# malcolmgreaves/deequ

Hardware: AMD Instinct MI355X
Metric: rows/sec (whole node) for fused 16-col profile scan; % of HBM peak BW (higher is better)
Workload: dtype f64+int64+utf8; 1 GPU; C5 fused 16-col profile scan (8 f64 + 4 i64 + 4 utf8, 10% nulls) + state merge + incremental StateLoader append; rows_per_gpu=1000000000, chunk_rows=125000000, analyzers=93, parallelism=row-shard x1

## Files before the change

### deequ_amd/csrc/dq_kernels.hip

```cpp
#include <hip/hip_runtime.h>

#include <cstdint>
#include <type_traits>

#include "dq_device.h"
#include "dq_hash.h"
#include "dq_decimal.h"
#include "dq_lane.h"
#include "dq_shift.h"

namespace dq {

#define DQ_DEC_TABLE static __constant__ const
#include "dq_dec_tables.inc"
#undef DQ_DEC_TABLE
__device__ __forceinline__ DecTab dec_dev_tab() { return DecTab{kDecP10Lo, kDecP10Hi, kDecRcpHi, kDecRcpLo}; }

typedef uint32_t u32x4 __attribute__((ext_vector_type(4)));

__device__ __forceinline__ uint32_t ld32(const uint8_t* base, int64_t a) {
  return *reinterpret_cast<const uint32_t*>(base + a);
}
__device__ __forceinline__ uint32_t read4(const uint8_t* base, int64_t pos) {
  int64_t a = pos & ~int64_t(3);
// ... 60 lines not shown

__device__ __forceinline__ void hll_update_if(int32_t* regs, uint64_t x, bool b) {
  atomicMax(&regs[(uint32_t)(x >> 55)], b ? hll_q_exact(x) : -1);
}

__device__ __forceinline__ int32_t ffbh_raw(uint32_t x) {
  int32_t r;
  asm("v_ffbh_u32 %0, %1" : "=v"(r) : "v"(x));
  return r;
}

struct HllKey {
  uint32_t addr;
  int32_t q;
};
__device__ __forceinline__ HllKey hll_key_from_fmix(uint64_t b) {
  const uint32_t bl = (uint32_t)b, bh = (uint32_t)(b >> 32);
  const uint32_t hi = __umulhi(bl, (uint32_t)XP3) + bl * (uint32_t)(XP3 >> 32) + bh * (uint32_t)XP3;
  return {(hi >> 21) & 0x7FCu, ffbh_raw(hi << 9)};
}
__device__ __forceinline__ HllKey hll_key_long(uint64_t v) { return hll_key_from_fmix(xxh64_long_head(v)); }
__device__ __forceinline__ HllKey hll_key_int(uint32_t v) { return hll_key_from_fmix(xxh64_int_head(v)); }


struct ColStats {
  double n, mean, m2, sum;
  int64_t isum, count, nan_count;
  double fmin, fmax;
  int64_t pinf, ninf;
  int64_t isum_hi;
};

__device__ __forceinline__ void stats_init(ColStats& s) {
  s.n = 0.0; s.mean = 0.0; s.m2 = 0.0; s.sum = 0.0;
// ... 170 lines not shown
    asm volatile(
        "s_and_saveexec_b64 %[save], %[ma]\n\t"
        "v_add_f64 %[d], %[x], -%[sh]\n\t"
        "v_add_f64 %[sd], %[sd], %[d]\n\t"
        "v_fma_f64 %[sdd], %[d], %[d], %[sdd]\n\t"
        "s_and_b64 exec, %[save], %[mb]\n\t"
        "v_min_f64 %[lo], %[lo], %[x]\n\t"
        "v_max_f64 %[hi], %[hi], %[x]\n\t"
        "s_mov_b64 exec, %[save]"
        : [sd] "+v"(a.sd), [sdd] "+v"(a.sdd), [lo] "+v"(lo), [hi] "+v"(hi), [d] "=&v"(d), [save] "=&s"(save)
        : [x] "v"(x), [sh] "s"(shift), [ma] "s"(ma), [mb] "s"(mb)
        : "scc");
  }
}

template <int KIND, bool STATS, bool HLL>
__device__ __forceinline__ void numeric_block(const double (&x)[8], const uint64_t (&bits)[8], const uint64_t (&m)[8],
                                              double shift, ColStats& s, LaneMoments& a, int32_t* regs, int32_t& qmin) {
#pragma unroll
  for (int j = 0; j < 8; ++j) {
    if (STATS) masked_moments<!ck_float(KIND), false>(a, s.fmin, s.fmax, x[j], bits[j], shift, m[j], m[j]);
    if (HLL) {
      const HllKey key = ck_bytes(KIND) <= 4 ? hll_key_int((uint32_t)bits[j]) : hll_key_long(bits[j]);
      qmin = min(qmin, key.q);
      if (lane_bit(m[j])) atomicMax(reinterpret_cast<int32_t*>(reinterpret_cast<char*>(regs) + key.addr), key.q);
    }
  }
  if (HLL) {
    if (__builtin_amdgcn_ballot_w64(qmin < 0) != 0) {
#pragma unroll 1
      for (int j = 0; j < 8; ++j) {
        if (lane_bit(m[j])) hll_update(regs, ck_bytes(KIND) <= 4 ? xxh64_int((uint32_t)bits[j]) : xxh64_long(bits[j]));
      }
      qmin = 0;
    }
  }
}

template <int KIND, bool STATS, bool HLL>
__device__ __forceinline__ void float_block_checked(__amdgpu_buffer_rsrc_t vr, const uint32_t* validity,
                                                    const uint32_t* mask, int64_t base, int32_t rem, int32_t vo,
                                                    double shift, ColStats& s, LaneMoments& a, int32_t* regs,
                                                    int64_t& cnt_w, int64_t& nan_v, int64_t& pinf_v, int64_t& ninf_v) {
  constexpr bool kF32 = KIND == CK_F32;
// ... 36 lines not shown
        else hll_update(regs, kF32 ? xxh64_int((uint32_t)b) : xxh64_long(b));
      }
    }
  }
}

template <int K> struct KindT { using T = double; };
template <> struct KindT<CK_I64> { using T = int64_t; };
template <> struct KindT<CK_I32> { using T = int32_t; };
template <> struct KindT<CK_F32> { using T = float; };
template <> struct KindT<CK_I16> { using T = int16_t; };
template <> struct KindT<CK_I8> { using T = int8_t; };

template <int KIND, bool STATS, bool HLL>
__device__ void numeric_range(const void* values, const uint32_t* validity, const uint32_t* mask,
                              int64_t row0, int64_t row1, ColStats& s, int32_t* regs) {
  using T = typename KindT<KIND>::T;
  constexpr bool kLazy = ck_float(KIND) && STATS;
  const int lane = threadIdx.x & 63;
  const int wave = __builtin_amdgcn_readfirstlane(threadIdx.x >> 6);
  const T* v = reinterpret_cast<const T*>(values);
  const __amdgpu_buffer_rsrc_t vr = __builtin_amdgcn_make_buffer_rsrc(
      const_cast<T*>(v + row0), (short)0, (int)((row1 - row0) * (int64_t)sizeof(T)), 0x00020000);
  int64_t nan_v = 0, pinf_v = 0, ninf_v = 0;
  int64_t cnt_w = 0;
  LaneMoments a{0.0, 0.0, 0};
  const double shift =
      STATS ? range_shift(validity, mask, row0, row1, lane, [=](int64_t r) { return range_value<KIND>(vr, r - row0); }) : 0.0;
  int32_t qmin = 0;
  const int32_t nr = (int32_t)(row1 - row0);
  for (int32_t rb = 0; rb < nr; rb += kRowsPerIter) {
    const int64_t base = row0 + rb + wave * 512;
    const int32_t rem = nr - rb - wave * 512;
    const bool full = rb + kRowsPerIter <= nr;
    uint64_t bits[8], m[8];
    double x[8];
    const int32_t vo = (rb + wave * 512 + lane) * (int32_t)sizeof(T);
#pragma unroll
    for (int j = 0; j < 8; ++j) {
      if constexpr (sizeof(T) == 8) {
        const auto w2 = __builtin_amdgcn_raw_buffer_load_b64(vr, vo + j * 512, 0, 2 );
        bits[j] = ((uint64_t)w2[1] << 32) | w2[0];
        if (KIND == CK_F64) x[j] = __builtin_bit_cast(double, bits[j]);
        else x[j] = __builtin_fma((double)(int32_t)w2[1], 4294967296.0, (double)w2[0]);
      } else if constexpr (KIND == CK_F32) {
        const uint32_t w = __builtin_amdgcn_raw_buffer_load_b32(vr, vo + j * 256, 0, 2 );
        bits[j] = w;
        x[j] = (double)__builtin_bit_cast(float, w);
      } else {
        int32_t w;
        if constexpr (sizeof(T) == 4) w = (int32_t)__builtin_amdgcn_raw_buffer_load_b32(vr, vo + j * 256, 0, 2 );
        else if constexpr (sizeof(T) == 2) w = (int16_t)__builtin_amdgcn_raw_buffer_load_b16(vr, vo + j * 128, 0, 2 );
        else w = (int8_t)__builtin_amdgcn_raw_buffer_load_b8(vr, vo + j * 64, 0, 2 );
        bits[j] = (uint64_t)(int64_t)w;
        x[j] = (double)w;
      }
    }
    block_masks(validity, mask, base, rem, full, m);
    uint64_t nf_any = 0;
    if constexpr (ck_float(KIND) && !kLazy) {
#pragma unroll
      for (int j = 0; j < 8; ++j) nf_any |= __builtin_amdgcn_ballot_w64(!__builtin_isfinite(x[j])) & m[j];
    }
    if (ck_float(KIND) && !kLazy && nf_any != 0) {
      float_block_checked<KIND, STATS, HLL>(vr, validity, mask, base, rem, vo, shift, s, a, regs, cnt_w, nan_v, pinf_v,
                                            ninf_v);
    } else {
#pragma unroll
      for (int j = 0; j < 8; ++j) cnt_w += __builtin_popcountll(m[j]);
      numeric_block<KIND, STATS, HLL>(x, bits, m, shift, s, a, regs, qmin);
    }
  }
  if constexpr (kLazy) {
    __shared__ int32_t redo;
    if (threadIdx.x == 0) redo = 0;
    __syncthreads();
    const bool bad = !__builtin_isfinite(a.sd) || !__builtin_isfinite(a.sdd);
    if (__builtin_amdgcn_ballot_w64(bad) != 0 && lane == 0) redo = 1;
    __syncthreads();
    if (redo) {
      if (HLL) {
        for (int i = threadIdx.x; i < 512; i += kBlock) regs[i] = -1;
      }
      stats_init(s);
      a = LaneMoments{0.0, 0.0, 0};
      cnt_w = 0;
      __syncthreads();
// ... 599 lines not shown
    c += __popc(bits);
  }
  s.count += c;
}

template <int KIND, bool STATS, bool HLL>
__device__ void run_numeric(const ColTask& t, const ScanCols& cols, const ScanBitmaps& bm, int64_t row0, int64_t row1,
                            ColStats& s, int32_t* regs) {
  const uint32_t* mask = t.where >= 0 ? reinterpret_cast<const uint32_t*>(bm.where_bits[t.where]) : nullptr;
  numeric_range<KIND, STATS, HLL>(cols.values[t.col], cols.validity[t.col], mask, row0, row1, s, regs);
}

template <int V, bool LONG>
__device__ __forceinline__ void run_variant(const ColTask& t, const ScanCols& cols, const uint32_t* mask, int64_t row0,
                                            int64_t row1, int64_t n_rows, ColStats& s, int32_t* regs,
                                            const uint64_t* p5, uint32_t* dq, uint32_t* rare, uint32_t* cls) {
  const void* v = cols.values[t.col];
  const uint32_t* val = cols.validity[t.col];
  if constexpr (V == CV_VALIDITY) validity_range(val, mask, row0, row1, s);
  else if constexpr (V == CV_F64_S) numeric_range<CK_F64, true, false>(v, val, mask, row0, row1, s, regs);
  else if constexpr (V == CV_F64_SH) numeric_range<CK_F64, true, true>(v, val, mask, row0, row1, s, regs);
  else if constexpr (V == CV_F64_H) numeric_range<CK_F64, false, true>(v, val, mask, row0, row1, s, regs);
  else if constexpr (V == CV_I64_S) numeric_range<CK_I64, true, false>(v, val, mask, row0, row1, s, regs);
  else if constexpr (V == CV_I64_SH) numeric_range<CK_I64, true, true>(v, val, mask, row0, row1, s, regs);
  else if constexpr (V == CV_I64_H) numeric_range<CK_I64, false, true>(v, val, mask, row0, row1, s, regs);
  else if constexpr (V == CV_I32_S) numeric_range<CK_I32, true, false>(v, val, mask, row0, row1, s, regs);
  else if constexpr (V == CV_I32_SH) numeric_range<CK_I32, true, true>(v, val, mask, row0, row1, s, regs);
  else if constexpr (V == CV_I32_H) numeric_range<CK_I32, false, true>(v, val, mask, row0, row1, s, regs);
  else if constexpr (V == CV_F32_S) numeric_range<CK_F32, true, false>(v, val, mask, row0, row1, s, regs);
  else if constexpr (V == CV_F32_SH) numeric_range<CK_F32, true, true>(v, val, mask, row0, row1, s, regs);
  else if constexpr (V == CV_F32_H) numeric_range<CK_F32, false, true>(v, val, mask, row0, row1, s, regs);
  else if constexpr (V == CV_I16_S) numeric_range<CK_I16, true, false>(v, val, mask, row0, row1, s, regs);
  else if constexpr (V == CV_I16_SH) numeric_range<CK_I16, true, true>(v, val, mask, row0, row1, s, regs);
  else if constexpr (V == CV_I16_H) numeric_range<CK_I16, false, true>(v, val, mask, row0, row1, s, regs);
  else if constexpr (V == CV_I8_S) numeric_range<CK_I8, true, false>(v, val, mask, row0, row1, s, regs);
  else if constexpr (V == CV_I8_SH) numeric_range<CK_I8, true, true>(v, val, mask, row0, row1, s, regs);
  else if constexpr (V == CV_I8_H) numeric_range<CK_I8, false, true>(v, val, mask, row0, row1, s, regs);
  else if constexpr (V == CV_F64_D) float_dtype_range(reinterpret_cast<const double*>(v), val, mask, row0, row1, s);
  else if constexpr (V == CV_F32_D) float_dtype_range(reinterpret_cast<const float*>(v), val, mask, row0, row1, s);
  else if constexpr (V == CV_BOOL) bool_range(reinterpret_cast<const uint32_t*>(v), val, mask, row0, row1, s, regs);
  else if constexpr (V == CV_D128_S) decimal_range<true, false, false>(v, val, mask, row0, row1, s, regs, t.arg);
  else if constexpr (V == CV_D128_SH) decimal_range<true, true, false>(v, val, mask, row0, row1, s, regs, t.arg);
  else if constexpr (V == CV_D128_H) decimal_range<false, true, false>(v, val, mask, row0, row1, s, regs, t.arg);
  else if constexpr (V == CV_D128_D) decimal_range<false, false, true>(v, val, mask, row0, row1, s, regs, t.arg);
  else if constexpr (V == CV_UTF8_H || V == CV_UTF8_D || V == CV_UTF8_HD)
    utf8_range<int32_t, V != CV_UTF8_D, V != CV_UTF8_H, LONG>(
        reinterpret_cast<const uint8_t*>(v), reinterpret_cast<const int32_t*>(cols.offsets[t.col]), val, mask, row0,
        row1, n_rows, s, regs, p5, dq, rare, cls);
  else
    utf8_range<int64_t, V != CV_LUTF8_D, V != CV_LUTF8_H, LONG>(
        reinterpret_cast<const uint8_t*>(v), reinterpret_cast<const int64_t*>(cols.offsets[t.col]), val, mask, row0,
        row1, n_rows, s, regs, p5, dq, rare, cls);
// ... 5 lines not shown
#ifndef DQ_NUM_WAVES
#define DQ_NUM_WAVES 6
#endif
template <int V, bool LONG>
constexpr int kMinWaves = V == CV_UTF8_H && !LONG && DQ_STR_CLS ? 5
                          : V == CV_UTF8_H && DQ_STR_WAVES > 0 ? DQ_STR_WAVES
                          : (V == CV_F64_SH || V == CV_I64_SH) && DQ_NUM_WAVES > 0 ? DQ_NUM_WAVES
                          : V == CV_LUTF8_H && LONG ? 5
                                                    : 1;

template <int V, bool LONG = false>
__global__ __launch_bounds__(kBlock) __attribute__((amdgpu_waves_per_eu(kMinWaves<V, LONG>))) void dq_column_scan(const ColTask* __restrict__ tasks, int32_t ntasks,
                                                         int32_t part_base, ScanCols cols, ScanBitmaps bm,
                                                         int64_t n_rows, int64_t rows_per_range,
                                                         ColPartial* __restrict__ partials,
                                                         uint32_t* __restrict__ hll_acc) {
  constexpr bool kHll = !(V == CV_VALIDITY || V == CV_F64_S || V == CV_I64_S || V == CV_I32_S || V == CV_F64_D ||
                         V == CV_UTF8_D || V == CV_LUTF8_D || V == CV_F32_S || V == CV_I16_S || V == CV_I8_S ||
                         V == CV_F32_D || V == CV_BOOL || V == CV_D128_S || V == CV_D128_D);
  constexpr bool kBool = V == CV_BOOL;
  constexpr bool kStr = V == CV_UTF8_H || V == CV_LUTF8_H || V == CV_UTF8_HD || V == CV_LUTF8_HD;
  __shared__ int32_t regs[kHll ? 512 : 2];
  __shared__ uint64_t p5[kStr ? 256 : 1];
  constexpr uint32_t kDCap = DQ_STR_CLS && (V == CV_UTF8_H || V == CV_LUTF8_H) && !LONG ? kDefCapCls : kDefCap;
  __shared__ uint32_t dfq[kStr ? kWaves * kDefFields * kDCap : 1];
  __shared__ uint32_t rare[kStr ? kWaves : 1];
  constexpr bool kCls = DQ_STR_CLS && (V == CV_UTF8_H || V == CV_LUTF8_H) && !LONG;
  __shared__ __attribute__((aligned(16))) uint32_t clsbuf[kCls ? kWaves * kClsWords : 4];
  __shared__ ColStats red[kWaves];
  const int32_t ti = blockIdx.x % ntasks;
  const int32_t range = blockIdx.x / ntasks;
// ... 6 lines not shown
    __syncthreads();
  }
  if constexpr (kHll) {
    for (int i = threadIdx.x; i < 512; i += kBlock) regs[i] = -1;
    if constexpr (kStr) {
      p5[threadIdx.x] = (uint64_t)threadIdx.x * XP5;
      if (threadIdx.x < kWaves) rare[threadIdx.x] = 0;
    }
    __syncthreads();
  }
  ColStats s;
  stats_init(s);
  const uint32_t* mask = t.where >= 0 ? reinterpret_cast<const uint32_t*>(bm.where_bits[t.where]) : nullptr;
  const int32_t wv = kStr ? __builtin_amdgcn_readfirstlane(threadIdx.x >> 6) : 0;
  run_variant<V, LONG>(t, cols, mask, row0, row1, n_rows, s, regs, p5, dfq + wv * kDefFields * kDCap, rare + wv,
                       clsbuf + (kCls ? wv * kClsWords : 0));
  block_reduce_store(s, partials + (size_t)(part_base + ti) * kMaxWG + range, red);
  if constexpr (kStr) {
    if (threadIdx.x == 0 && bm.rare_rows) {
      uint32_t r = 0;
      for (int w = 0; w < kWaves; ++w) r += rare[w];
      if (r) atomicAdd(reinterpret_cast<unsigned long long*>(bm.rare_rows + part_base + ti), (unsigned long long)r);
    }
  }
  if constexpr (kBool) {
    if (threadIdx.x == 0 && t.hll_slot >= 0) {
      uint32_t* dst = hll_acc + ((size_t)t.hll_slot * kHllCopies + (blockIdx.x % kHllCopies)) * 512;
      for (int b = 0; b < 2; ++b) {
        if (!regs[b]) continue;
        const uint64_t x = xxh64_int(b == 0 ? 1u : 0u);
        atomicMax(dst + (uint32_t)(x >> 55), (uint32_t)(hll_q_exact(x) + 1));
// ... 505 lines not shown
        pred_logic_op(ow, S, sp, lane);
      }
    }
    pred_block_out(S, s_ctr, n_counters, s_bmroot, n_bitmaps, bm, wr, inr, n_rows, lane);
  }
  pred_counters_out(pred_lds, wave_words, prog, acc);
}

__global__ __launch_bounds__(kBlock) void dq_finalize(int32_t ncol, int32_t nranges_col,
                                                      const ColPartial* __restrict__ col_part,
                                                      ColPartial* __restrict__ col_acc, int32_t npair, int32_t nranges_pair,
                                                      const CorrPartial* __restrict__ pair_part,
                                                      CorrPartial* __restrict__ pair_acc, int32_t has_pred,
                                                      int32_t nranges_pred, const PredPartial* __restrict__ pred_part,
                                                      PredPartial* __restrict__ pred_acc, FinRanges fr,
                                                      int64_t* __restrict__ rare_dev, int64_t* rare_host) {
  __shared__ ColStats cs[kBlock];
  __shared__ CorrStats ps[kBlock];
  const int b = blockIdx.x, tid = threadIdx.x;
  if (b < ncol) {
    int32_t nr = nranges_col;
    for (int i = 0; i < fr.n; ++i)
      if (b >= fr.first[i] && b < fr.end[i]) nr = fr.nr[i];
    ColStats s;
    stats_init(s);
    for (int r = tid; r < nr; r += kBlock) stats_merge(s, stats_load(col_part + (size_t)b * kMaxWG + r));
    cs[tid] = s;
    __syncthreads();
    for (int stride = kBlock / 2; stride >= 1; stride >>= 1) {
      if (tid < stride) { ColStats a = cs[tid]; stats_merge(a, cs[tid + stride]); cs[tid] = a; }
      __syncthreads();
// ... 15 lines not shown
      CorrStats o = {q.n, q.xa, q.ya, q.ck, q.xm, q.ym};
      corr_merge(s, o);
    }
    ps[tid] = s;
    __syncthreads();
    for (int stride = kBlock / 2; stride >= 1; stride >>= 1) {
      if (tid < stride) { CorrStats a = ps[tid]; corr_merge(a, ps[tid + stride]); ps[tid] = a; }
      __syncthreads();
    }
    if (tid == 0) {
      CorrPartial& q = pair_acc[p];
      CorrStats acc = {q.n, q.xa, q.ya, q.ck, q.xm, q.ym};
      corr_merge(acc, ps[0]);
      q.n = acc.n; q.xa = acc.xa; q.ya = acc.ya; q.ck = acc.ck; q.xm = acc.xm; q.ym = acc.ym;
    }
  } else if (has_pred) {
    static_assert(kBlock % kMaxCounters == 0, "counter layout");
    constexpr int G = kBlock / kMaxCounters;
    __shared__ int64_t st[G][kMaxCounters], sn[G][kMaxCounters];
    const int c = tid % kMaxCounters, g = tid / kMaxCounters;
    int64_t t = 0, nn = 0;
    for (int r = g; r < nranges_pred; r += G) { t += pred_part[r].t[c]; nn += pred_part[r].nn[c]; }
    st[g][c] = t;
    sn[g][c] = nn;
    __syncthreads();
    if (tid < kMaxCounters) {
      int64_t a = pred_acc->t[tid], b = pred_acc->nn[tid];
      for (int k = 0; k < G; ++k) { a += st[k][tid]; b += sn[k][tid]; }
      pred_acc->t[tid] = a;
      pred_acc->nn[tid] = b;
// ... 18 lines not shown
hipError_t launch_pred_scan(const PredProgram* prog, const ScanCols& cols, const ScanBitmaps& bm, int64_t n_rows,
                            int64_t rows_per_range, int32_t nranges, PredPartial* acc, int32_t lds_bytes, hipStream_t st,
                            bool has_regex) {
  if (has_regex)
    hipLaunchKernelGGL(dq_pred_scan<true>, dim3(nranges), dim3(kBlock), (size_t)lds_bytes, st, prog, cols, bm, n_rows,
                       rows_per_range, acc);
  else
    hipLaunchKernelGGL(dq_pred_scan<false>, dim3(nranges), dim3(kBlock), (size_t)lds_bytes, st, prog, cols, bm, n_rows,
                       rows_per_range, acc);
  return hipGetLastError();
}

template <int V>
static void launch_v(const ColTask* tasks, int32_t ntasks, int32_t part_base, const ScanCols& cols,
                     const ScanBitmaps& bm, int64_t n_rows, int64_t rows_per_range, int32_t nranges,
                     ColPartial* partials, uint32_t* hll_acc, bool long_str, hipStream_t st) {
  constexpr bool kStrHll = V == CV_UTF8_H || V == CV_LUTF8_H || V == CV_UTF8_HD || V == CV_LUTF8_HD;
  if constexpr (kStrHll) {
    if (long_str) {
      hipLaunchKernelGGL((dq_column_scan<V, true>), dim3((uint32_t)ntasks * (uint32_t)nranges), dim3(kBlock), 0, st,
                         tasks, ntasks, part_base, cols, bm, n_rows, rows_per_range, partials, hll_acc);
      return;
    }
  }
  hipLaunchKernelGGL(dq_column_scan<V>, dim3((uint32_t)ntasks * (uint32_t)nranges), dim3(kBlock), 0, st, tasks, ntasks,
                     part_base, cols, bm, n_rows, rows_per_range, partials, hll_acc);
}

hipError_t launch_column_scan(int32_t variant, const ColTask* tasks, int32_t ntasks, int32_t part_base,
                              const ScanCols& cols, const ScanBitmaps& bm, int64_t n_rows, int64_t rows_per_range,
                              int32_t nranges, ColPartial* partials, uint32_t* hll_acc, bool long_str, hipStream_t st) {
#define DQ_V(V)                                                                                            \
  case V:                                                                                                  \
    launch_v<V>(tasks, ntasks, part_base, cols, bm, n_rows, rows_per_range, nranges, partials, hll_acc, long_str, \
                st);                                                                                       \
    break;
  switch (variant) {
    DQ_V(CV_VALIDITY) DQ_V(CV_F64_S) DQ_V(CV_F64_SH) DQ_V(CV_F64_H) DQ_V(CV_I64_S) DQ_V(CV_I64_SH) DQ_V(CV_I64_H)
    DQ_V(CV_I32_S) DQ_V(CV_I32_SH) DQ_V(CV_I32_H) DQ_V(CV_UTF8_H) DQ_V(CV_LUTF8_H)
    DQ_V(CV_UTF8_D) DQ_V(CV_UTF8_HD) DQ_V(CV_LUTF8_D) DQ_V(CV_LUTF8_HD) DQ_V(CV_F64_D)
    DQ_V(CV_F32_S) DQ_V(CV_F32_SH) DQ_V(CV_F32_H) DQ_V(CV_I16_S) DQ_V(CV_I16_SH) DQ_V(CV_I16_H)
    DQ_V(CV_I8_S) DQ_V(CV_I8_SH) DQ_V(CV_I8_H) DQ_V(CV_F32_D) DQ_V(CV_BOOL)
    DQ_V(CV_D128_S) DQ_V(CV_D128_SH) DQ_V(CV_D128_H) DQ_V(CV_D128_D)
    default: return hipErrorInvalidValue;
  }
#undef DQ_V
  return hipGetLastError();
}


hipError_t launch_finalize(int32_t ncol, int32_t nranges_col, const ColPartial* col_part, ColPartial* col_acc,
                           int32_t npair, int32_t nranges_pair, const CorrPartial* pair_part, CorrPartial* pair_acc,
                           int32_t has_pred, int32_t nranges_pred, const PredPartial* pred_part, PredPartial* pred_acc,
                           const FinRanges& fr, int64_t* rare_dev, int64_t* rare_host, hipStream_t st) {
  const uint32_t nb = (uint32_t)(ncol + npair + (has_pred ? 1 : 0));
  if (nb == 0) return hipSuccess;
  hipLaunchKernelGGL(dq_finalize, dim3(nb), dim3(kBlock), 0, st, ncol, nranges_col, col_part, col_acc, npair,
                     nranges_pair, pair_part, pair_acc, has_pred, nranges_pred, pred_part, pred_acc, fr, rare_dev,
                     rare_host);
  return hipGetLastError();
}

hipError_t launch_init_acc(ColPartial* col_acc, int32_t ncol, CorrPartial* pair_acc, int32_t npair, int64_t* rare_dev,
                           hipStream_t st) {
  const int n = ncol > npair ? ncol : npair;
  if (n == 0) return hipSuccess;
  hipLaunchKernelGGL(dq_init_acc, dim3((n + 255) / 256), dim3(256), 0, st, col_acc, ncol, pair_acc, npair, rare_dev);
  return hipGetLastError();
}

}
```

### deequ_amd/csrc/dq_plan.cpp

```cpp
#include <hip/hip_runtime.h>

#include <algorithm>
#include <chrono>
#include <cmath>
#include <cstdarg>
#include <cstdio>
#include <cstdlib>
#include <cstring>
#include <functional>
#include <iterator>
#include <limits>
#include <map>
#include <memory>
#include <string>
#include <tuple>
#include <vector>

#include "dq_device.h"
#include "dq_internal.h"
#include "dq_pred_jit.h"

#ifndef DQ_MIN_RANGE_ROWS
#define DQ_MIN_RANGE_ROWS 16384
#endif
// ... 6 lines not shown
#ifndef DQ_PAIR_ONE_ROUND
#define DQ_PAIR_ONE_ROUND 1
#endif
#ifndef DQ_PRED_WGS
#define DQ_PRED_WGS 2048
#endif
#include "dq_regex.h"

namespace dq {

hipError_t launch_pred_scan(const PredProgram* prog, const ScanCols& cols, const ScanBitmaps& bm, int64_t n_rows,
                            int64_t rows_per_range, int32_t nranges, PredPartial* acc, int32_t lds_bytes, hipStream_t st,
                            bool has_regex);
hipError_t launch_column_scan(int32_t variant, const ColTask* tasks, int32_t ntasks, int32_t part_base,
                              const ScanCols& cols, const ScanBitmaps& bm, int64_t n_rows, int64_t rows_per_range,
                              int32_t nranges, ColPartial* partials, uint32_t* hll_acc, bool long_str, hipStream_t st);
hipError_t launch_pair_scan(const PairWG* wgs, int32_t nwg, const ScanCols& cols, const ScanBitmaps& bm,
                            const uint32_t* ones, int64_t n_rows, int64_t rows_per_range, int32_t nranges,
                            CorrPartial* pair_part, ColPartial* col_part, int32_t* redo, bool all_f64, bool ring,
                            bool minmax, hipStream_t st);
hipError_t pair_scan_residency(bool all_f64, bool ring, bool minmax, int32_t* per_cu);
hipError_t launch_finalize(int32_t ncol, int32_t nranges_col, const ColPartial* col_part, ColPartial* col_acc,
                           int32_t npair, int32_t nranges_pair, const CorrPartial* pair_part, CorrPartial* pair_acc,
                           int32_t has_pred, int32_t nranges_pred, const PredPartial* pred_part, PredPartial* pred_acc, const FinRanges& fr, int64_t* rare_dev, int64_t* rare_host,
                           hipStream_t st);
hipError_t launch_init_acc(ColPartial* col_acc, int32_t ncol, CorrPartial* pair_acc, int32_t npair, int64_t* rare_dev,
                           hipStream_t st);

static thread_local char g_err[1024] = "";
static thread_local bool g_capacity = false;

dq_status set_error(dq_status code, const char* fmt, ...) {
  va_list ap;
  va_start(ap, fmt);
  std::vsnprintf(g_err, sizeof(g_err), fmt, ap);
  va_end(ap);
  return code;
}

static dq_status cap_error(const char* fmt, ...) {
// ... 546 lines not shown
  int32_t* d_pair_redo = nullptr;
  char* h_stage = nullptr;
  int64_t* d_rare_dev = nullptr;
  int64_t* h_rare = nullptr;
  int64_t* d_rare = nullptr;
  std::vector<uint8_t> str_long;
  int32_t str_path = 0;
  int64_t prev_rows = 0;
  size_t h_stage_bytes = 0;
  PredProgram* d_prog = nullptr;
  ColPartial* d_col_part = nullptr;
  CorrPartial* d_pair_part = nullptr;
  PredPartial* d_pred_part = nullptr;
  ColPartial* d_col_acc = nullptr;
  uint32_t* d_hll_acc = nullptr;
  CorrPartial* d_pair_acc = nullptr;
  PredPartial* d_pred_acc = nullptr;
  uint64_t* d_where_bits[kMaxWhere] = {nullptr};
  int64_t where_cap_words = 0;
  uint32_t* d_ones = nullptr;
  int64_t ones_cap_words = 0;

  int64_t total_rows = 0;
  int64_t next_chunk = 0;

  bool timing = false;
  std::vector<hipEvent_t> ev_pool;
  struct Pending { int kernel; hipEvent_t a, b; };
  std::vector<Pending> pending;
  static constexpr int kTimers = 16 + kNumVariants;
// ... 40 lines not shown
  HIP_TRY(fn());
  if (p->timing) {
    HIP_TRY(hipEventRecord(b, st));
    p->pending.push_back({kernel, a, b});
  }
  return DQ_OK;
}

static dq_status free_plan_mem(dq_plan* p) {
  for (auto& q : p->pending) { p->ev_pool.push_back(q.a); p->ev_pool.push_back(q.b); }
  p->pending.clear();
  for (hipEvent_t e : p->ev_pool) (void)hipEventDestroy(e);
  p->ev_pool.clear();
  void* ptrs[] = {p->d_col_tasks, p->d_pair_tasks, p->d_pair_wgs, p->d_prog, p->d_col_part, p->d_pair_part,
                  p->d_pred_part, p->d_col_acc, p->d_hll_acc, p->d_pair_acc, p->d_pred_acc, p->d_regex, p->d_pair_redo,
                  p->d_rare_dev};
  for (void* q : ptrs)
    if (q) (void)hipFree(q);
  for (int i = 0; i < kMaxWhere; ++i)
    if (p->d_where_bits[i]) (void)hipFree(p->d_where_bits[i]);
  if (p->d_ones) (void)hipFree(p->d_ones);
  if (p->h_rare) (void)hipHostFree(p->h_rare);
  p->h_rare = p->d_rare = nullptr;
  if (p->h_stage) (void)hipHostFree(p->h_stage);
  p->h_stage = nullptr;
  p->h_stage_bytes = 0;
  return DQ_OK;
}

static dq_status reset_acc(dq_plan* p) {
  HIP_TRY(launch_init_acc(p->d_col_acc, (int32_t)p->col_tasks.size(), p->d_pair_acc, (int32_t)p->pair_tasks.size(),
                          p->d_rare_dev, p->stream));
  if (p->n_hll) HIP_TRY(hipMemsetAsync(p->d_hll_acc, 0, (size_t)p->n_hll * kHllCopies * 512 * sizeof(uint32_t), p->stream));
  if (p->has_pred) HIP_TRY(hipMemsetAsync(p->d_pred_acc, 0, kPredAccCopies * sizeof(PredPartial), p->stream));
  if (p->total_rows > 0) p->prev_rows = p->total_rows;
  p->total_rows = 0;
  p->next_chunk = 0;
  return DQ_OK;
}

template <typename T>
static dq_status dmalloc(T** ptr, size_t bytes) {
  if (bytes == 0) bytes = 16;
  HIP_TRY(hipMalloc((void**)ptr, bytes));
  return DQ_OK;
}

static void plan_pair_wgs(const dq_plan* p, const PairGroup& g, std::vector<PairWG>& out, std::vector<int>& fused) {
// ... 519 lines not shown
  if (nct) HIP_TRY(hipMemsetAsync(p->d_rare_dev, 0, 2 * nct * sizeof(int64_t), p->stream));
  p->str_long.assign(nct, 0);
  if (const char* e = std::getenv("DQ_STR_PATH")) p->str_path = std::strcmp(e, "fast") == 0 ? 1 : std::strcmp(e, "long") == 0 ? 2 : 0;
  if (nct && hipHostMalloc(reinterpret_cast<void**>(&p->h_rare), nct * sizeof(int64_t), hipHostMallocMapped) == hipSuccess) {
    std::memset(p->h_rare, 0, nct * sizeof(int64_t));
    void* dp = nullptr;
    if (hipHostGetDevicePointer(&dp, p->h_rare, 0) == hipSuccess) {
      p->d_rare = static_cast<int64_t*>(dp);
    } else {
      (void)hipHostFree(p->h_rare);
      p->h_rare = nullptr;
    }
  }
  (void)hipGetLastError();
  if (dq_status s = dmalloc(&p->d_hll_acc, (size_t)p->n_hll * kHllCopies * 512 * sizeof(uint32_t))) return s;
  if (dq_status s = dmalloc(&p->d_pair_acc, npt * sizeof(CorrPartial))) return s;
  if (dq_status s = dmalloc(&p->d_pred_acc, kPredAccCopies * sizeof(PredPartial))) return s;
  if (nct) HIP_TRY(hipMemcpyAsync(p->d_col_tasks, p->col_tasks.data(), nct * sizeof(ColTask), hipMemcpyHostToDevice, p->stream));
  if (npt) HIP_TRY(hipMemcpyAsync(p->d_pair_tasks, p->pair_tasks.data(), npt * sizeof(PairTask), hipMemcpyHostToDevice, p->stream));
  if (!p->regex_blob.empty()) {
    if (dq_status s = dmalloc(&p->d_regex, p->regex_blob.size() * sizeof(uint16_t))) return s;
    HIP_TRY(hipMemcpyAsync(p->d_regex, p->regex_blob.data(), p->regex_blob.size() * sizeof(uint16_t),
                           hipMemcpyHostToDevice, p->stream));
  }
  p->prog.regex = p->d_regex;
  p->prog.regex_words = (int32_t)p->regex_blob.size();
  HIP_TRY(hipMemcpyAsync(p->d_prog, &p->prog, sizeof(PredProgram), hipMemcpyHostToDevice, p->stream));
  if (dq_status s = reset_acc(p)) return s;
  HIP_TRY(hipStreamSynchronize(p->stream));
  return DQ_OK;
// ... 521 lines not shown
    if (g.variant != CV_UTF8_H && g.variant != CV_LUTF8_H && g.variant != CV_UTF8_HD && g.variant != CV_LUTF8_HD)
      return false;
    if (p->str_path != 0) return p->str_path == 2;
    const int64_t rows = p->total_rows > 0 ? p->total_rows : p->prev_rows;
    bool any = false;
    for (int32_t t = g.first; t < g.first + g.count; ++t) {
      if (p->h_rare && rows > 0) p->str_long[t] = __atomic_load_n(p->h_rare + t, __ATOMIC_RELAXED) * 4096 > rows;
      any = any || p->str_long[t];
    }
    return any;
  };
  for (size_t gi = 0; gi < groups.size(); ++gi) {
    const auto& g = groups[gi];
    if (dq_status s = timed(p, 16 + g.variant, p->stream, [&] {
          return launch_column_scan(g.variant, p->d_col_tasks + g.first, g.count, g.first, sc, bm, n_rows,
                                    vr[gi].first, vr[gi].second, p->d_col_part, p->d_hll_acc, str_long_of(g),
                                    p->stream);
        }))
      return s;
  }
  if (!p->pair_wgs.empty()) {
    const bool ring = pair_ring;
    if (dq_status s = timed(p, 2, p->stream, [&] {
          return launch_pair_scan(p->d_pair_wgs, (int32_t)p->pair_wgs.size(), sc, bm, p->d_ones, n_rows, rpr_pair,
                                  nr_pair, p->d_pair_part, p->d_col_part, p->d_pair_redo, p->pair_all_f64, ring,
                                  p->pair_minmax, p->stream);
        }))
      return s;
  }
  if (dq_status s = timed(p, 3, p->stream, [&] {
        return launch_finalize((int32_t)p->col_tasks.size(), nr_col, p->d_col_part, p->d_col_acc,
                               (int32_t)p->pair_tasks.size(), nr_pair, p->d_pair_part, p->d_pair_acc,
                               0 , nr_pred, p->d_pred_part, p->d_pred_acc,
                               fr, p->d_rare_dev, p->d_rare, p->stream);
      }))
    return s;
  p->total_rows += n_rows;
  return DQ_OK;
}

dq_status dq_finish(dq_plan* p, dq_state* out) {
  if (!p) return set_error(DQ_E_INVALID, "dq_finish: plan is NULL");
  if (!out && !p->specs.empty()) return set_error(DQ_E_INVALID, "dq_finish: out is NULL");
  HIP_TRY(hipSetDevice(p->device));
  if (!p->parts.empty()) {
    std::vector<dq_state> tmp;
    for (size_t k = 0; k < p->parts.size(); ++k) {
      tmp.assign(p->part_specs[k].size(), dq_state{});
      if (dq_status s = dq_finish(p->parts[k], tmp.data())) return s;
// ... 404 lines not shown
```

Measured before the change: 29.50 billion rows/s.

## Skip HLL register atomics when hash rank cannot exceed accumulated register floor

After each chunk, the finalize kernel now computes a per-sketch floor, the minimum register value across all 512 HLL registers. The next chunk's numeric scans use that floor as a threshold. While the floor is high enough, each lane only hashes its values and tracks the minimum shifted hash. The atomicMax updates run only when some lane could raise a register. This removes almost all HLL atomics on later chunks of an incremental scan, at the cost of an extra finalize block per sketch and a second specialised loop body with more code.

After: 30.01 billion rows/s (median of 6 runs). 1.02x the previous value.

```diff
diff --git a/deequ_amd/csrc/dq_kernels.hip b/deequ_amd/csrc/dq_kernels.hip
--- a/deequ_amd/csrc/dq_kernels.hip
+++ b/deequ_amd/csrc/dq_kernels.hip
@@ -98,10 +98,20 @@
   uint32_t addr;
   int32_t q;
 };
+__device__ __forceinline__ uint32_t hll_hi_from_fmix(uint64_t b) {
+  const uint32_t bl = (uint32_t)b, bh = (uint32_t)(b >> 32);
+  return __umulhi(bl, (uint32_t)XP3) + bl * (uint32_t)(XP3 >> 32) + bh * (uint32_t)XP3;
+}
 __device__ __forceinline__ HllKey hll_key_from_fmix(uint64_t b) {
-  const uint32_t bl = (uint32_t)b, bh = (uint32_t)(b >> 32);
-  const uint32_t hi = __umulhi(bl, (uint32_t)XP3) + bl * (uint32_t)(XP3 >> 32) + bh * (uint32_t)XP3;
+  const uint32_t hi = hll_hi_from_fmix(b);
   return {(hi >> 21) & 0x7FCu, ffbh_raw(hi << 9)};
+}
+
+constexpr int32_t kFloorMin = 13;
+__device__ __forceinline__ uint32_t hll_floor_thr(const uint32_t* __restrict__ hll_floor, int32_t slot) {
+  if (!hll_floor || slot < 0) return 0u;
+  const int32_t qfloor = (int32_t)hll_floor[slot] - 1;
+  return qfloor >= kFloorMin ? 1u << (31 - min(qfloor, 22)) : 0u;
 }
 __device__ __forceinline__ HllKey hll_key_long(uint64_t v) { return hll_key_from_fmix(xxh64_long_head(v)); }
 __device__ __forceinline__ HllKey hll_key_int(uint32_t v) { return hll_key_from_fmix(xxh64_int_head(v)); }
@@ -302,20 +312,28 @@
   }
 }
 
-template <int KIND, bool STATS, bool HLL>
+template <int KIND, bool STATS, bool HLL, bool FLOOR = false>
 __device__ __forceinline__ void numeric_block(const double (&x)[8], const uint64_t (&bits)[8], const uint64_t (&m)[8],
-                                              double shift, ColStats& s, LaneMoments& a, int32_t* regs, int32_t& qmin) {
+                                              double shift, ColStats& s, LaneMoments& a, int32_t* regs, int32_t& qmin,
+                                              uint32_t thr = 0) {
+  uint32_t rmin = ~0u;
 #pragma unroll
   for (int j = 0; j < 8; ++j) {
     if (STATS) masked_moments<!ck_float(KIND), false>(a, s.fmin, s.fmax, x[j], bits[j], shift, m[j], m[j]);
     if (HLL) {
-      const HllKey key = ck_bytes(KIND) <= 4 ? hll_key_int((uint32_t)bits[j]) : hll_key_long(bits[j]);
-      qmin = min(qmin, key.q);
-      if (lane_bit(m[j])) atomicMax(reinterpret_cast<int32_t*>(reinterpret_cast<char*>(regs) + key.addr), key.q);
+      if constexpr (FLOOR) {
+        const uint64_t b = ck_bytes(KIND) <= 4 ? xxh64_int_head((uint32_t)bits[j]) : xxh64_long_head(bits[j]);
+        rmin = min(rmin, hll_hi_from_fmix(b) << 9);
+      } else {
+        const HllKey key = ck_bytes(KIND) <= 4 ? hll_key_int((uint32_t)bits[j]) : hll_key_long(bits[j]);
+        qmin = min(qmin, key.q);
+        if (lane_bit(m[j])) atomicMax(reinterpret_cast<int32_t*>(reinterpret_cast<char*>(regs) + key.addr), key.q);
+      }
     }
   }
   if (HLL) {
-    if (__builtin_amdgcn_ballot_w64(qmin < 0) != 0) {
+    const bool redo = FLOOR ? rmin < thr : qmin < 0;
+    if (__builtin_amdgcn_ballot_w64(redo) != 0) {
 #pragma unroll 1
       for (int j = 0; j < 8; ++j) {
         if (lane_bit(m[j])) hll_update(regs, ck_bytes(KIND) <= 4 ? xxh64_int((uint32_t)bits[j]) : xxh64_long(bits[j]));
@@ -382,7 +400,7 @@
 
 template <int KIND, bool STATS, bool HLL>
 __device__ void numeric_range(const void* values, const uint32_t* validity, const uint32_t* mask,
-                              int64_t row0, int64_t row1, ColStats& s, int32_t* regs) {
+                              int64_t row0, int64_t row1, ColStats& s, int32_t* regs, uint32_t thr = 0) {
   using T = typename KindT<KIND>::T;
   constexpr bool kLazy = ck_float(KIND) && STATS;
   const int lane = threadIdx.x & 63;
@@ -397,48 +415,53 @@
       STATS ? range_shift(validity, mask, row0, row1, lane, [=](int64_t r) { return range_value<KIND>(vr, r - row0); }) : 0.0;
   int32_t qmin = 0;
   const int32_t nr = (int32_t)(row1 - row0);
-  for (int32_t rb = 0; rb < nr; rb += kRowsPerIter) {
-    const int64_t base = row0 + rb + wave * 512;
-    const int32_t rem = nr - rb - wave * 512;
-    const bool full = rb + kRowsPerIter <= nr;
-    uint64_t bits[8], m[8];
-    double x[8];
-    const int32_t vo = (rb + wave * 512 + lane) * (int32_t)sizeof(T);
-#pragma unroll
-    for (int j = 0; j < 8; ++j) {
-      if constexpr (sizeof(T) == 8) {
-        const auto w2 = __builtin_amdgcn_raw_buffer_load_b64(vr, vo + j * 512, 0, 2 );
-        bits[j] = ((uint64_t)w2[1] << 32) | w2[0];
-        if (KIND == CK_F64) x[j] = __builtin_bit_cast(double, bits[j]);
-        else x[j] = __builtin_fma((double)(int32_t)w2[1], 4294967296.0, (double)w2[0]);
-      } else if constexpr (KIND == CK_F32) {
-        const uint32_t w = __builtin_amdgcn_raw_buffer_load_b32(vr, vo + j * 256, 0, 2 );
-        bits[j] = w;
-        x[j] = (double)__builtin_bit_cast(float, w);
+  auto block_loop = [&](auto floor_form) __attribute__((always_inline)) {
+    constexpr bool FLOOR = decltype(floor_form)::value;
+    for (int32_t rb = 0; rb < nr; rb += kRowsPerIter) {
+      const int64_t base = row0 + rb + wave * 512;
+      const int32_t rem = nr - rb - wave * 512;
+      const bool full = rb + kRowsPerIter <= nr;
+      uint64_t bits[8], m[8];
+      double x[8];
+      const int32_t vo = (rb + wave * 512 + lane) * (int32_t)sizeof(T);
+#pragma unroll
+      for (int j = 0; j < 8; ++j) {
+        if constexpr (sizeof(T) == 8) {
+          const auto w2 = __builtin_amdgcn_raw_buffer_load_b64(vr, vo + j * 512, 0, 2 );
+          bits[j] = ((uint64_t)w2[1] << 32) | w2[0];
+          if (KIND == CK_F64) x[j] = __builtin_bit_cast(double, bits[j]);
+          else x[j] = __builtin_fma((double)(int32_t)w2[1], 4294967296.0, (double)w2[0]);
+        } else if constexpr (KIND == CK_F32) {
+          const uint32_t w = __builtin_amdgcn_raw_buffer_load_b32(vr, vo + j * 256, 0, 2 );
+          bits[j] = w;
+          x[j] = (double)__builtin_bit_cast(float, w);
+        } else {
+          int32_t w;
+          if constexpr (sizeof(T) == 4) w = (int32_t)__builtin_amdgcn_raw_buffer_load_b32(vr, vo + j * 256, 0, 2 );
+          else if constexpr (sizeof(T) == 2) w = (int16_t)__builtin_amdgcn_raw_buffer_load_b16(vr, vo + j * 128, 0, 2 );
+          else w = (int8_t)__builtin_amdgcn_raw_buffer_load_b8(vr, vo + j * 64, 0, 2 );
+          bits[j] = (uint64_t)(int64_t)w;
+          x[j] = (double)w;
+        }
+      }
+      block_masks(validity, mask, base, rem, full, m);
+      uint64_t nf_any = 0;
+      if constexpr (ck_float(KIND) && !kLazy) {
+#pragma unroll
+        for (int j = 0; j < 8; ++j) nf_any |= __builtin_amdgcn_ballot_w64(!__builtin_isfinite(x[j])) & m[j];
+      }
+      if (ck_float(KIND) && !kLazy && nf_any != 0) {
+        float_block_checked<KIND, STATS, HLL>(vr, validity, mask, base, rem, vo, shift, s, a, regs, cnt_w, nan_v, pinf_v,
+                                              ninf_v);
       } else {
-        int32_t w;
-        if constexpr (sizeof(T) == 4) w = (int32_t)__builtin_amdgcn_raw_buffer_load_b32(vr, vo + j * 256, 0, 2 );
-        else if constexpr (sizeof(T) == 2) w = (int16_t)__builtin_amdgcn_raw_buffer_load_b16(vr, vo + j * 128, 0, 2 );
-        else w = (int8_t)__builtin_amdgcn_raw_buffer_load_b8(vr, vo + j * 64, 0, 2 );
-        bits[j] = (uint64_t)(int64_t)w;
-        x[j] = (double)w;
-      }
-    }
-    block_masks(validity, mask, base, rem, full, m);
-    uint64_t nf_any = 0;
-    if constexpr (ck_float(KIND) && !kLazy) {
-#pragma unroll
-      for (int j = 0; j < 8; ++j) nf_any |= __builtin_amdgcn_ballot_w64(!__builtin_isfinite(x[j])) & m[j];
-    }
-    if (ck_float(KIND) && !kLazy && nf_any != 0) {
-      float_block_checked<KIND, STATS, HLL>(vr, validity, mask, base, rem, vo, shift, s, a, regs, cnt_w, nan_v, pinf_v,
-                                            ninf_v);
-    } else {
-#pragma unroll
-      for (int j = 0; j < 8; ++j) cnt_w += __builtin_popcountll(m[j]);
-      numeric_block<KIND, STATS, HLL>(x, bits, m, shift, s, a, regs, qmin);
-    }
-  }
+#pragma unroll
+        for (int j = 0; j < 8; ++j) cnt_w += __builtin_popcountll(m[j]);
+        numeric_block<KIND, STATS, HLL, FLOOR>(x, bits, m, shift, s, a, regs, qmin, thr);
+      }
+    }
+  };
+  if (HLL && thr != 0) block_loop(std::true_type{});
+  else block_loop(std::false_type{});
   if constexpr (kLazy) {
     __shared__ int32_t redo;
     if (threadIdx.x == 0) redo = 0;
@@ -1068,28 +1091,29 @@
 template <int V, bool LONG>
 __device__ __forceinline__ void run_variant(const ColTask& t, const ScanCols& cols, const uint32_t* mask, int64_t row0,
                                             int64_t row1, int64_t n_rows, ColStats& s, int32_t* regs,
-                                            const uint64_t* p5, uint32_t* dq, uint32_t* rare, uint32_t* cls) {
+                                            const uint64_t* p5, uint32_t* dq, uint32_t* rare, uint32_t* cls,
+                                            uint32_t thr) {
   const void* v = cols.values[t.col];
   const uint32_t* val = cols.validity[t.col];
   if constexpr (V == CV_VALIDITY) validity_range(val, mask, row0, row1, s);
   else if constexpr (V == CV_F64_S) numeric_range<CK_F64, true, false>(v, val, mask, row0, row1, s, regs);
-  else if constexpr (V == CV_F64_SH) numeric_range<CK_F64, true, true>(v, val, mask, row0, row1, s, regs);
-  else if constexpr (V == CV_F64_H) numeric_range<CK_F64, false, true>(v, val, mask, row0, row1, s, regs);
+  else if constexpr (V == CV_F64_SH) numeric_range<CK_F64, true, true>(v, val, mask, row0, row1, s, regs, thr);
+  else if constexpr (V == CV_F64_H) numeric_range<CK_F64, false, true>(v, val, mask, row0, row1, s, regs, thr);
   else if constexpr (V == CV_I64_S) numeric_range<CK_I64, true, false>(v, val, mask, row0, row1, s, regs);
-  else if constexpr (V == CV_I64_SH) numeric_range<CK_I64, true, true>(v, val, mask, row0, row1, s, regs);
-  else if constexpr (V == CV_I64_H) numeric_range<CK_I64, false, true>(v, val, mask, row0, row1, s, regs);
+  else if constexpr (V == CV_I64_SH) numeric_range<CK_I64, true, true>(v, val, mask, row0, row1, s, regs, thr);
+  else if constexpr (V == CV_I64_H) numeric_range<CK_I64, false, true>(v, val, mask, row0, row1, s, regs, thr);
   else if constexpr (V == CV_I32_S) numeric_range<CK_I32, true, false>(v, val, mask, row0, row1, s, regs);
-  else if constexpr (V == CV_I32_SH) numeric_range<CK_I32, true, true>(v, val, mask, row0, row1, s, regs);
-  else if constexpr (V == CV_I32_H) numeric_range<CK_I32, false, true>(v, val, mask, row0, row1, s, regs);
+  else if constexpr (V == CV_I32_SH) numeric_range<CK_I32, true, true>(v, val, mask, row0, row1, s, regs, thr);
+  else if constexpr (V == CV_I32_H) numeric_range<CK_I32, false, true>(v, val, mask, row0, row1, s, regs, thr);
   else if constexpr (V == CV_F32_S) numeric_range<CK_F32, true, false>(v, val, mask, row0, row1, s, regs);
-  else if constexpr (V == CV_F32_SH) numeric_range<CK_F32, true, true>(v, val, mask, row0, row1, s, regs);
-  else if constexpr (V == CV_F32_H) numeric_range<CK_F32, false, true>(v, val, mask, row0, row1, s, regs);
+  else if constexpr (V == CV_F32_SH) numeric_range<CK_F32, true, true>(v, val, mask, row0, row1, s, regs, thr);
+  else if constexpr (V == CV_F32_H) numeric_range<CK_F32, false, true>(v, val, mask, row0, row1, s, regs, thr);
   else if constexpr (V == CV_I16_S) numeric_range<CK_I16, true, false>(v, val, mask, row0, row1, s, regs);
-  else if constexpr (V == CV_I16_SH) numeric_range<CK_I16, true, true>(v, val, mask, row0, row1, s, regs);
-  else if constexpr (V == CV_I16_H) numeric_range<CK_I16, false, true>(v, val, mask, row0, row1, s, regs);
+  else if constexpr (V == CV_I16_SH) numeric_range<CK_I16, true, true>(v, val, mask, row0, row1, s, regs, thr);
+  else if constexpr (V == CV_I16_H) numeric_range<CK_I16, false, true>(v, val, mask, row0, row1, s, regs, thr);
   else if constexpr (V == CV_I8_S) numeric_range<CK_I8, true, false>(v, val, mask, row0, row1, s, regs);
-  else if constexpr (V == CV_I8_SH) numeric_range<CK_I8, true, true>(v, val, mask, row0, row1, s, regs);
-  else if constexpr (V == CV_I8_H) numeric_range<CK_I8, false, true>(v, val, mask, row0, row1, s, regs);
+  else if constexpr (V == CV_I8_SH) numeric_range<CK_I8, true, true>(v, val, mask, row0, row1, s, regs, thr);
+  else if constexpr (V == CV_I8_H) numeric_range<CK_I8, false, true>(v, val, mask, row0, row1, s, regs, thr);
   else if constexpr (V == CV_F64_D) float_dtype_range(reinterpret_cast<const double*>(v), val, mask, row0, row1, s);
   else if constexpr (V == CV_F32_D) float_dtype_range(reinterpret_cast<const float*>(v), val, mask, row0, row1, s);
   else if constexpr (V == CV_BOOL) bool_range(reinterpret_cast<const uint32_t*>(v), val, mask, row0, row1, s, regs);
@@ -1125,7 +1149,8 @@
                                                          int32_t part_base, ScanCols cols, ScanBitmaps bm,
                                                          int64_t n_rows, int64_t rows_per_range,
                                                          ColPartial* __restrict__ partials,
-                                                         uint32_t* __restrict__ hll_acc) {
+                                                         uint32_t* __restrict__ hll_acc,
+                                                         const uint32_t* __restrict__ hll_floor) {
   constexpr bool kHll = !(V == CV_VALIDITY || V == CV_F64_S || V == CV_I64_S || V == CV_I32_S || V == CV_F64_D ||
                          V == CV_UTF8_D || V == CV_LUTF8_D || V == CV_F32_S || V == CV_I16_S || V == CV_I8_S ||
                          V == CV_F32_D || V == CV_BOOL || V == CV_D128_S || V == CV_D128_D);
@@ -1162,7 +1187,7 @@
   const uint32_t* mask = t.where >= 0 ? reinterpret_cast<const uint32_t*>(bm.where_bits[t.where]) : nullptr;
   const int32_t wv = kStr ? __builtin_amdgcn_readfirstlane(threadIdx.x >> 6) : 0;
   run_variant<V, LONG>(t, cols, mask, row0, row1, n_rows, s, regs, p5, dfq + wv * kDefFields * kDCap, rare + wv,
-                       clsbuf + (kCls ? wv * kClsWords : 0));
+                       clsbuf + (kCls ? wv * kClsWords : 0), kHll ? hll_floor_thr(hll_floor, t.hll_slot) : 0u);
   block_reduce_store(s, partials + (size_t)(part_base + ti) * kMaxWG + range, red);
   if constexpr (kStr) {
     if (threadIdx.x == 0 && bm.rare_rows) {
@@ -1698,7 +1723,9 @@
                                                       CorrPartial* __restrict__ pair_acc, int32_t has_pred,
                                                       int32_t nranges_pred, const PredPartial* __restrict__ pred_part,
                                                       PredPartial* __restrict__ pred_acc, FinRanges fr,
-                                                      int64_t* __restrict__ rare_dev, int64_t* rare_host) {
+                                                      int64_t* __restrict__ rare_dev, int64_t* rare_host,
+                                                      int32_t nhll, const uint32_t* __restrict__ hll_acc,
+                                                      uint32_t* __restrict__ hll_floor) {
   __shared__ ColStats cs[kBlock];
   __shared__ CorrStats ps[kBlock];
   const int b = blockIdx.x, tid = threadIdx.x;
@@ -1744,6 +1771,24 @@
       corr_merge(acc, ps[0]);
       q.n = acc.n; q.xa = acc.xa; q.ya = acc.ya; q.ck = acc.ck; q.xm = acc.xm; q.ym = acc.ym;
     }
+  } else if (b >= ncol + npair + (has_pred ? 1 : 0)) {
+    const int slot = b - (ncol + npair + (has_pred ? 1 : 0));
+    if (slot >= nhll) return;
+    __shared__ uint32_t fmin_w[kWaves];
+    const uint32_t* src = hll_acc + (size_t)slot * kHllCopies * 512;
+    uint32_t f = ~0u;
+    for (int i = tid; i < 512; i += kBlock) {
+      uint32_t r = 0;
+      for (int c = 0; c < kHllCopies; ++c) r = max(r, src[c * 512 + i]);
+      f = min(f, r);
+    }
+    for (int o = 32; o >= 1; o >>= 1) f = min(f, (uint32_t)__shfl_xor((int)f, o));
+    if ((tid & 63) == 0) fmin_w[tid >> 6] = f;
+    __syncthreads();
+    if (tid == 0) {
+      for (int w = 1; w < kWaves; ++w) f = min(f, fmin_w[w]);
+      hll_floor[slot] = f;
+    }
   } else if (has_pred) {
     static_assert(kBlock % kMaxCounters == 0, "counter layout");
     constexpr int G = kBlock / kMaxCounters;
@@ -1792,26 +1837,28 @@
 template <int V>
 static void launch_v(const ColTask* tasks, int32_t ntasks, int32_t part_base, const ScanCols& cols,
                      const ScanBitmaps& bm, int64_t n_rows, int64_t rows_per_range, int32_t nranges,
-                     ColPartial* partials, uint32_t* hll_acc, bool long_str, hipStream_t st) {
+                     ColPartial* partials, uint32_t* hll_acc, const uint32_t* hll_floor, bool long_str,
+                     hipStream_t st) {
   constexpr bool kStrHll = V == CV_UTF8_H || V == CV_LUTF8_H || V == CV_UTF8_HD || V == CV_LUTF8_HD;
   if constexpr (kStrHll) {
     if (long_str) {
       hipLaunchKernelGGL((dq_column_scan<V, true>), dim3((uint32_t)ntasks * (uint32_t)nranges), dim3(kBlock), 0, st,
-                         tasks, ntasks, part_base, cols, bm, n_rows, rows_per_range, partials, hll_acc);
+                         tasks, ntasks, part_base, cols, bm, n_rows, rows_per_range, partials, hll_acc, hll_floor);
       return;
     }
   }
   hipLaunchKernelGGL(dq_column_scan<V>, dim3((uint32_t)ntasks * (uint32_t)nranges), dim3(kBlock), 0, st, tasks, ntasks,
-                     part_base, cols, bm, n_rows, rows_per_range, partials, hll_acc);
+                     part_base, cols, bm, n_rows, rows_per_range, partials, hll_acc, hll_floor);
 }
 
 hipError_t launch_column_scan(int32_t variant, const ColTask* tasks, int32_t ntasks, int32_t part_base,
                               const ScanCols& cols, const ScanBitmaps& bm, int64_t n_rows, int64_t rows_per_range,
-                              int32_t nranges, ColPartial* partials, uint32_t* hll_acc, bool long_str, hipStream_t st) {
+                              int32_t nranges, ColPartial* partials, uint32_t* hll_acc, const uint32_t* hll_floor,
+                              bool long_str, hipStream_t st) {
 #define DQ_V(V)                                                                                            \
   case V:                                                                                                  \
-    launch_v<V>(tasks, ntasks, part_base, cols, bm, n_rows, rows_per_range, nranges, partials, hll_acc, long_str, \
-                st);                                                                                       \
+    launch_v<V>(tasks, ntasks, part_base, cols, bm, n_rows, rows_per_range, nranges, partials, hll_acc, hll_floor, \
+                long_str, st);                                                                             \
     break;
   switch (variant) {
     DQ_V(CV_VALIDITY) DQ_V(CV_F64_S) DQ_V(CV_F64_SH) DQ_V(CV_F64_H) DQ_V(CV_I64_S) DQ_V(CV_I64_SH) DQ_V(CV_I64_H)
@@ -1830,12 +1877,14 @@
 hipError_t launch_finalize(int32_t ncol, int32_t nranges_col, const ColPartial* col_part, ColPartial* col_acc,
                            int32_t npair, int32_t nranges_pair, const CorrPartial* pair_part, CorrPartial* pair_acc,
                            int32_t has_pred, int32_t nranges_pred, const PredPartial* pred_part, PredPartial* pred_acc,
-                           const FinRanges& fr, int64_t* rare_dev, int64_t* rare_host, hipStream_t st) {
-  const uint32_t nb = (uint32_t)(ncol + npair + (has_pred ? 1 : 0));
+                           const FinRanges& fr, int64_t* rare_dev, int64_t* rare_host, int32_t nhll,
+                           const uint32_t* hll_acc, uint32_t* hll_floor, hipStream_t st) {
+  if (!hll_floor) nhll = 0;
+  const uint32_t nb = (uint32_t)(ncol + npair + (has_pred ? 1 : 0) + nhll);
   if (nb == 0) return hipSuccess;
   hipLaunchKernelGGL(dq_finalize, dim3(nb), dim3(kBlock), 0, st, ncol, nranges_col, col_part, col_acc, npair,
                      nranges_pair, pair_part, pair_acc, has_pred, nranges_pred, pred_part, pred_acc, fr, rare_dev,
-                     rare_host);
+                     rare_host, nhll, hll_acc, hll_floor);
   return hipGetLastError();
 }
 
diff --git a/deequ_amd/csrc/dq_plan.cpp b/deequ_amd/csrc/dq_plan.cpp
--- a/deequ_amd/csrc/dq_plan.cpp
+++ b/deequ_amd/csrc/dq_plan.cpp
@@ -44,7 +44,8 @@
                             bool has_regex);
 hipError_t launch_column_scan(int32_t variant, const ColTask* tasks, int32_t ntasks, int32_t part_base,
                               const ScanCols& cols, const ScanBitmaps& bm, int64_t n_rows, int64_t rows_per_range,
-                              int32_t nranges, ColPartial* partials, uint32_t* hll_acc, bool long_str, hipStream_t st);
+                              int32_t nranges, ColPartial* partials, uint32_t* hll_acc, const uint32_t* hll_floor,
+                              bool long_str, hipStream_t st);
 hipError_t launch_pair_scan(const PairWG* wgs, int32_t nwg, const ScanCols& cols, const ScanBitmaps& bm,
                             const uint32_t* ones, int64_t n_rows, int64_t rows_per_range, int32_t nranges,
                             CorrPartial* pair_part, ColPartial* col_part, int32_t* redo, bool all_f64, bool ring,
@@ -53,7 +54,7 @@
 hipError_t launch_finalize(int32_t ncol, int32_t nranges_col, const ColPartial* col_part, ColPartial* col_acc,
                            int32_t npair, int32_t nranges_pair, const CorrPartial* pair_part, CorrPartial* pair_acc,
                            int32_t has_pred, int32_t nranges_pred, const PredPartial* pred_part, PredPartial* pred_acc, const FinRanges& fr, int64_t* rare_dev, int64_t* rare_host,
-                           hipStream_t st);
+                           int32_t nhll, const uint32_t* hll_acc, uint32_t* hll_floor, hipStream_t st);
 hipError_t launch_init_acc(ColPartial* col_acc, int32_t ncol, CorrPartial* pair_acc, int32_t npair, int64_t* rare_dev,
                            hipStream_t st);
 
@@ -630,6 +631,7 @@
   PredPartial* d_pred_part = nullptr;
   ColPartial* d_col_acc = nullptr;
   uint32_t* d_hll_acc = nullptr;
+  uint32_t* d_hll_floor = nullptr;
   CorrPartial* d_pair_acc = nullptr;
   PredPartial* d_pred_acc = nullptr;
   uint64_t* d_where_bits[kMaxWhere] = {nullptr};
@@ -700,7 +702,7 @@
   p->ev_pool.clear();
   void* ptrs[] = {p->d_col_tasks, p->d_pair_tasks, p->d_pair_wgs, p->d_prog, p->d_col_part, p->d_pair_part,
                   p->d_pred_part, p->d_col_acc, p->d_hll_acc, p->d_pair_acc, p->d_pred_acc, p->d_regex, p->d_pair_redo,
-                  p->d_rare_dev};
+                  p->d_rare_dev, p->d_hll_floor};
   for (void* q : ptrs)
     if (q) (void)hipFree(q);
   for (int i = 0; i < kMaxWhere; ++i)
@@ -718,6 +720,7 @@
   HIP_TRY(launch_init_acc(p->d_col_acc, (int32_t)p->col_tasks.size(), p->d_pair_acc, (int32_t)p->pair_tasks.size(),
                           p->d_rare_dev, p->stream));
   if (p->n_hll) HIP_TRY(hipMemsetAsync(p->d_hll_acc, 0, (size_t)p->n_hll * kHllCopies * 512 * sizeof(uint32_t), p->stream));
+  if (p->n_hll && p->d_hll_floor) HIP_TRY(hipMemsetAsync(p->d_hll_floor, 0, (size_t)p->n_hll * sizeof(uint32_t), p->stream));
   if (p->has_pred) HIP_TRY(hipMemsetAsync(p->d_pred_acc, 0, kPredAccCopies * sizeof(PredPartial), p->stream));
   if (p->total_rows > 0) p->prev_rows = p->total_rows;
   p->total_rows = 0;
@@ -1267,6 +1270,9 @@
   }
   (void)hipGetLastError();
   if (dq_status s = dmalloc(&p->d_hll_acc, (size_t)p->n_hll * kHllCopies * 512 * sizeof(uint32_t))) return s;
+  const char* floor_env = std::getenv("DQ_HLL_FLOOR");
+  if (p->n_hll && !(floor_env && std::strcmp(floor_env, "0") == 0))
+    if (dq_status s = dmalloc(&p->d_hll_floor, (size_t)p->n_hll * sizeof(uint32_t))) return s;
   if (dq_status s = dmalloc(&p->d_pair_acc, npt * sizeof(CorrPartial))) return s;
   if (dq_status s = dmalloc(&p->d_pred_acc, kPredAccCopies * sizeof(PredPartial))) return s;
   if (nct) HIP_TRY(hipMemcpyAsync(p->d_col_tasks, p->col_tasks.data(), nct * sizeof(ColTask), hipMemcpyHostToDevice, p->stream));
@@ -1818,8 +1824,8 @@
     const auto& g = groups[gi];
     if (dq_status s = timed(p, 16 + g.variant, p->stream, [&] {
           return launch_column_scan(g.variant, p->d_col_tasks + g.first, g.count, g.first, sc, bm, n_rows,
-                                    vr[gi].first, vr[gi].second, p->d_col_part, p->d_hll_acc, str_long_of(g),
-                                    p->stream);
+                                    vr[gi].first, vr[gi].second, p->d_col_part, p->d_hll_acc, p->d_hll_floor,
+                                    str_long_of(g), p->stream);
         }))
       return s;
   }
@@ -1836,7 +1842,7 @@
         return launch_finalize((int32_t)p->col_tasks.size(), nr_col, p->d_col_part, p->d_col_acc,
                                (int32_t)p->pair_tasks.size(), nr_pair, p->d_pair_part, p->d_pair_acc,
                                0 , nr_pred, p->d_pred_part, p->d_pred_acc,
-                               fr, p->d_rare_dev, p->d_rare, p->stream);
+                               fr, p->d_rare_dev, p->d_rare, p->n_hll, p->d_hll_acc, p->d_hll_floor, p->stream);
       }))
     return s;
   p->total_rows += n_rows;
```
